# tahmidawal/Superresolution_for_PDEs

Measured on AMD Instinct MI355X. Metric: 20->40 SR training samples/sec at batch 1024 per GPU (fwd+MSE bwd+clip+AdamW), higher is better.
Workload: dtype f32 (h3: fp32 products from power-of-two-scaled 2-piece fp16 splits on fp16 MFMA, fp32 accumulate); 1 GPU; UNet 20->40 train step, fp32, batch 1024/GPU, 40x40; global_batch=1024, per_gpu_batch=1024, hw=40x40, parallelism=dp1

## Files before the change

include/srpde.h:

```cpp
#ifndef SRPDE_H_
#define SRPDE_H_

#include <stddef.h>

#ifdef __cplusplus
extern "C" {
#endif

typedef struct ihipStream_t* hipStream_t;

#define SRPDE_ABI_VERSION 17

#define SRPDE_FAM_NO_H5 2
#define SRPDE_FAM_NO_H4 4
#define SRPDE_FAM_NO_H3R 8

const char* srpde_last_error(void);
const char* srpde_last_kernel(void);
int srpde_version(void);

int srpde_pack_conv_weights(const float* w, float* wfwd, float* wdgrad, int cout, int cin, int cin_real,
                            int ksize, hipStream_t stream);
int srpde_conv_fwd(const float* x0, int c0, int ldx0, const float* x1, int c1, int ldx1, const float* wpack,
                   const float* bias, float* y, int ldy, int n, int h, int w, int cout, int ksize, int dil,
                   int sign, int accumulate, float* stats, const float* ep_mean, const float* ep_invstd,
                   const float* ep_gamma, const float* ep_beta, unsigned* ep_amax, void* workspace,
                   size_t ws_bytes, hipStream_t stream);
size_t srpde_conv_fwd_workspace_size(int cout);
size_t srpde_conv_stats_blocks(int n, int h, int w, int cout);
int srpde_conv_stats_rows_per_block(int cout);
size_t srpde_conv_wgrad_workspace_size(int n, int h, int w, int cout, int cin, int ksize);
int srpde_conv_wgrad(const float* dy, int lddy, const float* x0, int c0, int ldx0, const float* x1, int c1,
                     int ldx1, float* dw, int cin_real, int accumulate, int n, int h, int w, int cout, int ksize,
                     int dil, void* workspace, size_t ws_bytes, hipStream_t stream);
int srpde_conv_wgrad_bnb(const float* da, int ldda, const float* y, int ldy, const float* mean, const float* invstd,
                         const float* gamma, const float* beta, const float* m1, const float* m2, int flags,
                         const float* x0, int c0, int ldx0, float* dw, int cin_real, int accumulate, int n, int h,
                         int w, int cout, int ksize, int dil, void* workspace, size_t ws_bytes, hipStream_t stream);
int srpde_conv_h3_supported(int c0, int c1, int cout, int w, int dil, int ksize);
int srpde_conv_h3_stats_rows(void);
int srpde_conv_h3_stats_rows_for(int c0, int c1, int cout, int h, int w, int dil, int flags);
int srpde_split_weights_h3(const float* w, void* planes, int* wexp, int rows, int K, hipStream_t stream);
int srpde_absmax(const float* x, int ldx, int c, long long P, unsigned* amax, hipStream_t stream);
int srpde_prepare_weights_h3(const long long* desc, int nlayers, int total_rows, hipStream_t stream);
// ... 110 lines not shown
                                 const float* stats, int E, int S, int tile, float* x, hipStream_t stream);
int srpde_cascade_stitch_denorm(const float* y, const float* stats, int E, int S, int tile, double* u_next,
                                hipStream_t stream);
size_t srpde_field_metrics_workspace_size(int E, int n);
int srpde_field_metrics(const void* pred, int pred_is_f32, const double* gt, int E, int n, double* out,
                        void* workspace, size_t ws_bytes, hipStream_t stream);

int srpde_tiled_tiles_per_side(int S, int tile, int stride);
size_t srpde_tiled_level_stats_workspace_size(int E, int S);
int srpde_tiled_level_stats(const double* u_cur, const double* f_next, const double* theta_next, int E, int S,
                            float* stats, int* theta_const, void* workspace, size_t ws_bytes, hipStream_t stream);
int srpde_tiled_assemble(const double* u_cur, const double* f_next, const double* theta_next, const float* stats,
                         int E, int S, int tile, int stride, float* x, hipStream_t stream);
int srpde_tiled_blend_denorm(const float* y, const float* stats, int E, int S, int tile, int stride, int window,
                             double* u_next, hipStream_t stream);

int srpde_resize_bicubic_ac(const float* x, float* out, int planes, int h, int w, int ho, int wo,
                            hipStream_t stream);

int srpde_upsample_bilinear_fwd(const float* x, int ldx, float* out, int ldo, int n, int h, int w, int ho, int wo,
                                int c, hipStream_t stream);
int srpde_upsample_bilinear_bwd(const float* dout, int lddo, float* dx, int lddx, int n, int h, int w, int ho,
                                int wo, int c, int accumulate, hipStream_t stream);
int srpde_upsample_bilinear_gate_fwd(const float* x, int ldx, float* out, int ldo, int n, int h, int w, int ho,
                                      int wo, int c, const float* wg, const float* bg, float* sa, hipStream_t stream);
size_t srpde_upsample_gate_sa_workspace_size(int n, int h, int w);
int srpde_upsample_gate_sa(const float* x, int ldx, int n, int h, int w, int ho, int wo, int c, const float* wg,
                           const float* bg, float* sa, void* workspace, size_t ws_bytes, hipStream_t stream);
int srpde_conv_head_eval_supported(int w);
int srpde_conv_head_eval(const float* z, int ldz, const unsigned* amax_z, const void* wsplit, const int* wexp,
                         const float* bias, const float* bn_mean, const float* bn_invstd, const float* bn_gamma,
                         const float* bn_beta, const float* wf, const float* bf, const float* xin, int xin_c, int n,
                         int h, int w, float* out, hipStream_t stream);
int srpde_att_apply_fwd(const float* x, int ldx, int n, int hw, int c, const float* ca, const float* sa, float* out,
                        int ldo, hipStream_t stream);
int srpde_upsample_bilinear_bwd_gated(const float* dout, int lddo, const float* dsa, const float* wg, float* dx,
                                      int lddx, int n, int h, int w, int ho, int wo, int c, int accumulate,
                                      hipStream_t stream);
int srpde_gating_bn_reduce_blocks(long long P, int C);
int srpde_gating_bn_reduce(const float* dsa, const float* wg, float* dg, int lddg, const float* y, int ldy,
                           const float* mean, const float* invstd, const float* gamma, const float* beta, long long P,
                           int C, int flags, void* part, float* da_max, hipStream_t stream);
int srpde_upsample_bwd_bn_supported(int h, int w, int ho, int wo, int c, int lddo, int lddx);
int srpde_upsample_bilinear_bwd_gated_bn(const float* dout, int lddo, const float* dsa, const float* wg, float* dx,
                                         int lddx, int n, int h, int w, int ho, int wo, int c, const float* y, int ldy,
                                         const float* mean, const float* invstd, const float* gamma,
                                         const float* beta, int flags, void* part, float* da_max,
                                         hipStream_t stream);

int srpde_att_fwd(const float* x, int ldx, const float* g, int ldg, int n, int hw, int c, int gc, const float* w1,
                  const float* b1, const float* w2, const float* b2, const float* wg, const float* bg, float* m,
                  float* hbuf, float* ca, float* sa, float* out, int ldo, hipStream_t stream);
int srpde_att_channel_fwd(const float* x, int ldx, int n, int hw, int c, const float* w1, const float* b1,
                          const float* w2, const float* b2, float* m, float* hbuf, float* ca, hipStream_t stream);
int srpde_att_gate_fwd(const float* x, int ldx, const float* g, int ldg, int n, int hw, int c, int gc,
                       const float* ca, const float* wg, const float* bg, float* sa, float* out, int ldo,
                       hipStream_t stream);
size_t srpde_att_bwd_workspace_size(int n, int hw, int c, int gc);
int srpde_att_bwd(const float* dout, int lddo, const float* x, int ldx, const float* g, int ldg, int n, int hw,
                  int c, int gc, const float* w1, const float* w2, const float* wg, const float* m, const float* hbuf,
                  const float* ca, const float* sa, float* dx, int lddx, int dx_accumulate, float* dg, int lddg,
                  int dg_accumulate, float* dw1, float* db1, float* dw2, float* db2, float* dwg, float* dbg,
                  void* workspace, size_t ws_bytes, hipStream_t stream);
int srpde_att_pool_bn_bwd_blocks(int n, int h, int w, int c);
int srpde_att_pool_bn_bwd(const float* dout, int lddo, const float* ca, const float* sa, const float* dm, const float* a,
                          int lda, const float* dp, int lddp, const float* y, int ldy, const float* mean,
// ... 93 lines not shown
```

superresolution_for_pdes_amd/csrc/bn.hip:

```cpp
#include "bn_reduce.h"

namespace srpde {

struct Chan {
  double n, mean, m2;
};
__device__ __forceinline__ Chan chan_merge(Chan a, Chan b) {
  if (b.n == 0.0) return a;
  if (a.n == 0.0) return b;
  const double n = a.n + b.n, d = b.mean - a.mean;
  Chan r;
  r.n = n;
  r.mean = a.mean + d * (b.n / n);
  r.m2 = a.m2 + b.m2 + d * d * (a.n * b.n / n);
  return r;
}

__device__ __forceinline__ void fin_channel(int c, const float2* __restrict__ stats, int nblk, int nfull,
                                            int rows_per_blk, long long P, int C, double shift, double s1, double s2,
                                            double sm, float* running_mean, float* running_var, float momentum,
                                            float eps, float* __restrict__ mean_out, float* __restrict__ invstd_out,
                                            long long* num_batches_tracked, const float* __restrict__ gamma,
                                            const float* __restrict__ beta, float* __restrict__ scale_out,
                                            float* __restrict__ shift_out, unsigned* amax, float sqrt_pm1) {
// ... 306 lines not shown
      const float4 d = add4(scale4(dsa[p], w), old);
      st4(dg + p * lddg + c, d);
      acc.amax(d);
      acc.add(v, d, relu);
    };
    bn_rows(pb + r0, pe, rs, y, ldy, dg, lddg, c, row);
  }
  bn_bwd_block_combine(red4, threadIdx.x, (int)threadIdx.x < (C >> 2), threadIdx.x, C >> 2, rs, acc,
                       part + (size_t)blockIdx.x * C + c, true, da_max + blockIdx.x);
}

__global__ __launch_bounds__(256) void colsum2_kernel(const float2* __restrict__ part, int nblk, int C,
                                                      float* out0, float* out1, double* keep0, double* keep1) {
  const int c = blockIdx.x;
  __shared__ double a[256], b[256];
  double x = 0.0, yv = 0.0;
  for (int k = threadIdx.x; k < nblk; k += 256) {
    const float2 v = part[(size_t)k * C + c];
    x += v.x; yv += v.y;
  }
  a[threadIdx.x] = x; b[threadIdx.x] = yv;
  __syncthreads();
  for (int s = 128; s > 0; s >>= 1) {
    if ((int)threadIdx.x < s) { a[threadIdx.x] += a[threadIdx.x + s]; b[threadIdx.x] += b[threadIdx.x + s]; }
    __syncthreads();
  }
  if (threadIdx.x == 0) {
    if (out0) out0[c] = (float)a[0];
    if (out1) out1[c] = (float)b[0];
    if (keep0) keep0[c] = a[0];
    if (keep1) keep1[c] = b[0];
  }
}

struct BnBwdDy {
  float4 mu, is, g, b, m1, m2, k;
  __device__ __forceinline__ float dy1(float v, float mu1, float is1, float g1, float b1, float d, int relu, float a1,
                                       float a2, float k1) const {
    float xh;
    const float dz = bn_relu_mask(v, mu1, is1, g1, b1, d, relu, &xh);
    return (dz - a1 - xh * a2) * k1;
  }
  __device__ __forceinline__ float4 dy4(const float4& v, const float4& d, int relu) const {
    return make_float4(dy1(v.x, mu.x, is.x, g.x, b.x, d.x, relu, m1.x, m2.x, k.x),
                       dy1(v.y, mu.y, is.y, g.y, b.y, d.y, relu, m1.y, m2.y, k.y),
                       dy1(v.z, mu.z, is.z, g.z, b.z, d.z, relu, m1.z, m2.z, k.z),
                       dy1(v.w, mu.w, is.w, g.w, b.w, d.w, relu, m1.w, m2.w, k.w));
  }
};

__global__ __launch_bounds__(256) void bn_bwd_apply_kernel(const float* __restrict__ y, int ldy,
                                                           const float* __restrict__ da, int ldda,
                                                           const float* __restrict__ mean,
                                                           const float* __restrict__ invstd,
                                                           const float* __restrict__ gamma,
                                                           const float* __restrict__ beta,
                                                           const double* __restrict__ sdz,
                                                           const double* __restrict__ sdzx, long long P, int C,
                                                           int rows_per_blk, int relu, float* __restrict__ dy,
                                                           int lddy, float2* __restrict__ bias_part, unsigned* amax) {
  extern __shared__ float4 red4[];
  float mx = 0.f;
  int c4, r0, rs;
  thread_rc(C, &c4, &r0, &rs);
  const int active = (C >> 2) * rs;
  const int c = c4 * 4;
  float4 sb = zero4();
  if ((int)threadIdx.x < active) {
    const float4 mu = ld4(mean + c);
    const float4 is = ld4(invstd + c);
    const float4 g = ld4(gamma + c);
    const float4 b = ld4(beta + c);
    const double invP = (relu & 2) ? 0.0 : 1.0 / (double)P;
    float4 m1, m2, k;
    m1.x = (float)(sdz[c] * invP); m1.y = (float)(sdz[c + 1] * invP);
    m1.z = (float)(sdz[c + 2] * invP); m1.w = (float)(sdz[c + 3] * invP);
    m2.x = (float)(sdzx[c] * invP); m2.y = (float)(sdzx[c + 1] * invP);
    m2.z = (float)(sdzx[c + 2] * invP); m2.w = (float)(sdzx[c + 3] * invP);
    k.x = g.x * is.x; k.y = g.y * is.y; k.z = g.z * is.z; k.w = g.w * is.w;
    const long long pb = (long long)blockIdx.x * rows_per_blk;
    const long long pe = min(P, pb + rows_per_blk);
    const BnBwdDy f{mu, is, g, b, m1, m2, k};
// ... 639 lines not shown
```

superresolution_for_pdes_amd/csrc/bn_reduce.h:

```cpp
#pragma once
#include "vec4.h"

namespace srpde {

template <bool ALWAYS = false>
__device__ __forceinline__ float bn_relu_mask(float v, float mu, float is, float g, float b, float d, int relu,
                                              float* xhat) {
  const float xh = (v - mu) * is;
  *xhat = xh;
  return ((!ALWAYS && !(relu & 1)) || xh * g + b > 0.f) ? d : 0.f;
}

template <bool ALWAYS>
__device__ __forceinline__ void bn_bwd_add1(float v, float mu, float is, float g, float b, float d, int relu, float& t1,
                                            float& t2) {
  float xh;
  const float dz = bn_relu_mask<ALWAYS>(v, mu, is, g, b, d, relu, &xh);
  t1 += dz;
  t2 += dz * xh;
}

struct BnBwdAcc {
  float4 mu, is, g, b;
  float4 s1 = zero4(), s2 = zero4();
// ... 12 lines not shown
    bn_bwd_add1<ALWAYS>(y.y, mu.y, is.y, g.y, b.y, d.y, relu, s1.y, s2.y);
    bn_bwd_add1<ALWAYS>(y.z, mu.z, is.z, g.z, b.z, d.z, relu, s1.z, s2.z);
    bn_bwd_add1<ALWAYS>(y.w, mu.w, is.w, g.w, b.w, d.w, relu, s1.w, s2.w);
  }
  __device__ __forceinline__ void amax(const float4& d) { dmax = fmaxf(dmax, absmax4(d)); }
};

__device__ __forceinline__ void bn_bwd_store_part(const float4* sums, int C4, int nrows, int q, float2* o) {
  float4 t1 = zero4(), t2 = t1;
  for (int r = 0; r < nrows; ++r) {
    t1 = add4(t1, sums[r * C4 + q]);
    t2 = add4(t2, sums[256 + r * C4 + q]);
  }
  store_part4(o, t1, t2);
}
__device__ __forceinline__ float max4slots(const float* wmx) { return fmaxf(fmaxf(wmx[0], wmx[1]), fmaxf(wmx[2], wmx[3])); }

__device__ __forceinline__ void bn_bwd_block_combine(float4* red4, int tid, bool lead, int q, int C4, int nrows,
                                                     const BnBwdAcc& acc, float2* o, bool want_max, float* da_max) {
  red4[tid] = acc.s1;
  red4[256 + tid] = acc.s2;
  __syncthreads();
  if (lead) bn_bwd_store_part(red4, C4, nrows, q, o);
  if (want_max) {
    const float dmax = wave_max(acc.dmax);
    __syncthreads();
    float* wmx = reinterpret_cast<float*>(red4);
    if ((tid & 63) == 0) wmx[tid >> 6] = dmax;
    __syncthreads();
    if (tid == 0) *da_max = max4slots(wmx);
  }
}

}
```

superresolution_for_pdes_amd/csrc/conv_head.hip:

```cpp
#include "conv_h3.h"

namespace srpde {

struct HeadArgs {
  const float* z; int ldz;
  const unsigned* amax;
  const _Float16* wsp;
  const int* wexp;
  const float* bias;
  const float* mean; const float* invstd; const float* gamma; const float* beta;
  const float* wf; const float* bf;
  const float* xin; int xin_c;
  int N, H, W, P;
  float* out;
};

constexpr int HEAD_BM = 128, HEAD_SR = 160, HEAD_RB = HEAD_BM / 64;
constexpr int HEAD_IT = 4;

__global__ __launch_bounds__(256, 3) void conv_head_eval_kernel(HeadArgs a) {
  extern __shared__ __attribute__((aligned(16))) char lds[];
  const int tid = threadIdx.x, lane = tid & 63, wave = tid >> 6;
  const int l16 = lane & 15, lq = lane >> 4;
  const int W = a.W, HW = a.H * a.W, halo = W + 1, arows = HEAD_BM + 2 * halo;
  const int zrel = arows * HEAD_SR;
  const int m0 = blockIdx.x * HEAD_BM, pix0 = m0 - halo;
  const int ea = h3_exp(*a.amax);
  const float sa = exp2i(ea);

  half8 bh[9], bl[9];
#pragma unroll
  for (int t = 0; t < 9; ++t) {
    const size_t o = (size_t)l16 * 288 + t * 32 + lq * 8;
// ... 191 lines not shown
  float t = 0.f;
#pragma unroll
  for (int i = 0; i < HEAD_RB; ++i)
#pragma unroll
    for (int r = 0; r < 4; ++r) {
      const int px = m0 + wave * (16 * HEAD_RB) + i * 16 + lq * 4 + r;
      if (px < p.P) t += yv[i][r];
    }
  const float mean = chan_sum(t) / (float)cnt;
  t = 0.f;
#pragma unroll
  for (int i = 0; i < HEAD_RB; ++i)
#pragma unroll
    for (int r = 0; r < 4; ++r) {
      const int px = m0 + wave * (16 * HEAD_RB) + i * 16 + lq * 4 + r;
      const float d = yv[i][r] - mean;
      if (px < p.P) t = __builtin_fmaf(d, d, t);
    }
  const float m2 = chan_sum(t);
  if (tid < 16) p.stats[(size_t)blockIdx.x * 16 + tid] = make_float2(mean, m2);
}

bool n16_supported(int c0, int c1, int cout, int w, int dil) {
  return c0 == 32 && c1 == 0 && cout == 16 && dil == 1 && w > 0 && w <= 63 &&
         (size_t)(HEAD_BM + 2 * (w + 1)) * HEAD_SR + 128 + 256 <= 80 * 1024;
}

int launch_fwd_n16(const ConvParams& p, const H3Args& h, hipStream_t st) {
  const size_t lds = (size_t)(HEAD_BM + 2 * (p.W + 1)) * HEAD_SR + 128 + 256;
  note_kernel("conv_fwd_n16_kernel");
  hipLaunchKernelGGL(conv_fwd_n16_kernel, dim3(ceil_div(p.P, HEAD_BM)), dim3(256), lds, st, p, h);
  SRPDE_LAUNCH_CHECK("srpde_conv_fwd_h3(n16)");
  return 0;
}

}

using namespace srpde;

extern "C" {

int srpde_conv_head_eval_supported(int w) {
  return (w > 0 && w <= 63 && (size_t)(HEAD_BM + 2 * (w + 1)) * HEAD_SR + 128 <= 80 * 1024) ? 1 : 0;
}

int srpde_conv_head_eval(const float* z, int ldz, const unsigned* amax_z, const void* wsplit, const int* wexp,
                         const float* bias, const float* bn_mean, const float* bn_invstd, const float* bn_gamma,
                         const float* bn_beta, const float* wf, const float* bf, const float* xin, int xin_c, int n,
                         int h, int w, float* out, hipStream_t stream) {
  SRPDE_CHECK_ARG(z && amax_z && wsplit && wexp && bn_mean && bn_invstd && bn_gamma && bn_beta && wf && bf && xin &&
                      out && xin_c >= 1,
                  "srpde_conv_head_eval: null pointer");
  SRPDE_CHECK_ARG(n > 0 && h > 0 && w > 0 && (long long)n * h * w < (1LL << 31) && ldz % 4 == 0 && ldz >= 32 &&
                      aligned16(z) && aligned16(wsplit),
                  "srpde_conv_head_eval: bad shape / stride / alignment");
  HeadArgs a;
  a.z = z; a.ldz = ldz; a.amax = amax_z;
  a.wsp = static_cast<const _Float16*>(wsplit); a.wexp = wexp; a.bias = bias;
  a.mean = bn_mean; a.invstd = bn_invstd; a.gamma = bn_gamma; a.beta = bn_beta;
  a.wf = wf; a.bf = bf; a.xin = xin; a.xin_c = xin_c;
  a.N = n; a.H = h; a.W = w; a.P = n * h * w; a.out = out;
  const size_t lds = (size_t)(HEAD_BM + 2 * (w + 1)) * HEAD_SR + 128;
  SRPDE_CHECK_ARG(srpde_conv_head_eval_supported(w), "srpde_conv_head_eval: image rows too wide for the tile (w=%d > 63)",
                  w);
  note_kernel("conv_head_eval_kernel");
  hipLaunchKernelGGL(conv_head_eval_kernel, dim3(ceil_div(a.P, HEAD_BM)), dim3(256), lds, stream, a);
  SRPDE_LAUNCH_CHECK("srpde_conv_head_eval");
  return 0;
}

}
```

superresolution_for_pdes_amd/hipops.py:

```python
from __future__ import annotations

import os

import torch

from ._lib import call, last_error, query, stream_ptr

F32 = torch.float32


def _pl(t):
    assert t.dim() == 2 and (t.stride(1) == 1 or t.shape[1] == 1), "expected a [P, C] row-major view"
    assert t.dtype == F32 and t.is_cuda, "expected a CUDA fp32 tensor"
    return t.data_ptr(), t.stride(0)


def _p(t):
    return 0 if t is None else t.data_ptr()


def _pl_opt(t):
    return (0, 0, 0) if t is None else (*_pl(t), t.shape[1])


# ... 290 lines not shown
         beta.data_ptr(), P, C, flags, _p(part), part.shape[0] if part is not None else 0, _p(da_max),
         da_max.numel() if (part is not None) else 0, m1.data_ptr(), m2.data_ptr(), _p(dgamma), _p(dbeta), _p(dbias),
         word.data_ptr(), ws.data_ptr(), ws_bytes, stream_ptr())
    return m1, m2, word


def dx_max_slots(n, h, w, cin_dx, device):
    bn = 64 if cin_dx % 64 == 0 else 32
    return empty(-(-(n * h * w) // 256) * -(-cin_dx // bn), device=device)


def out_max_slots(n, h, w, cin, cout, dil, device):
    t = query("srpde_conv_h3_tiles", n * h * w, cin, cout, w, dil)
    assert t > 0, "out_max_slots: shape not on the h3 kernels"
    return empty(t, device=device)


def conv_dgrad_bnb(da, y, mean, invstd, gamma, beta, m1, m2, dy_amax, wpack, dx, n, h, w, cout_dy, cin_dx, dil,
                   dysplit, relu=True, bn_bwd=None, dx_max=None):
    planes, wexp = wpack.h3
    pda, ldda = _pl(da)
    py, ldy = _pl(y)
    pdx, lddx = _pl(dx)
    _check_rows(bn_bwd[5] if bn_bwd is not None else None, None, "the h3 kernel (bn_bwd_partials)")
    ws = _scratch(int(query("srpde_conv_fwd_workspace_size", cin_dx)), dx.device)
    _conv_call("srpde_conv_dgrad_h3_bnb", _conv_flop(cin_dx, cout_dy, 3, n, h, w), pda, ldda, dy_amax.data_ptr(), py,
               ldy, mean.data_ptr(), invstd.data_ptr(), gamma.data_ptr(), beta.data_ptr(), m1.data_ptr(),
               m2.data_ptr(), BN_RELU if relu else 0, planes.data_ptr(), wexp.data_ptr(), pdx, lddx, n, h, w, cout_dy,
               cin_dx, dil, dysplit.data_ptr(), *_bn_bwd_args(bn_bwd), _p(dx_max), ws.data_ptr(), ws.numel(),
               stream_ptr())
    dysplit._srpde_amax = dy_amax


def bn_bwd_partials(n, h, w, c, device):
    rows = int(query("srpde_conv_h3_stats_rows"))
    buf = empty(-(-(n * h * w) // rows), c, 2, device=device)
    buf._srpde_rows = rows
    return buf


class AmaxSlots:

    def __init__(self, n, device):
        self.buf = torch.zeros(n, dtype=torch.int32, device=device)
        self.next = 0
        self.eval_epilogue = False

    def take(self):
        if self.next >= self.buf.numel():
            raise RuntimeError("AmaxSlots exhausted")
        self.next += 1
        return self.buf[self.next - 1:self.next]


def tag_amax(t, slot):
    if slot is not None:
        t._srpde_amax = slot
    return t


def amax_of(x):
    a = getattr(x, "_srpde_amax", None)
    if a is None:
        a = torch.zeros(1, dtype=torch.int32, device=x.device)
        px, ld = _pl(x)
        call("srpde_absmax", px, ld, x.shape[1], x.shape[0], a.data_ptr(), stream_ptr())
# ... 735 lines not shown
```

superresolution_for_pdes_amd/unet_exec.py:

```python
from __future__ import annotations

import contextlib

import torch

from . import hipops as H

FORWARD_GROUPS = ["enc1", "enc2", "enc3", "bridge", "att3", "dec3", "att2", "dec2", "att1", "dec1",
                  "out_conv1", "out_bn1", "out_conv2", "out_bn2", "final"]
FLAT_GROUPS = list(reversed(FORWARD_GROUPS))


def flat_layout(model):
    named = dict(model.named_parameters())
    out, off = [], 0
    for grp in FLAT_GROUPS:
        for name, p in named.items():
            if name == grp or name.startswith(grp + "."):
                out.append((name, p, off, p.numel()))
                off += p.numel()
    assert off == sum(p.numel() for p in named.values()), "flat layout does not cover every parameter"
    return out


# ... 342 lines not shown
            fn()
        for t in keep:
            if t is not None:
                t.record_stream(self.side)

    def join(self):
        self.main.wait_stream(self.side)


_WGRAD_STREAM = True
_BWD_PRIORITY = "auto"
_PRIO_STREAMS = {}


def _priority_stream(dev):
    key = (dev.type, dev.index if dev.index is not None else torch.cuda.current_device())
    st = _PRIO_STREAMS.get(key)
    if st is None:
        lo, hi = torch.cuda.Stream.priority_range()
        st = _PRIO_STREAMS[key] = torch.cuda.Stream(device=dev, priority=hi)
    return st


def _xkeep(xp):
    return tuple(xp.tensors()) if isinstance(xp, H.XSource) else ()


def _bwd_path(saved, dx, dx_accumulate, cin, w, dil):
    x0, x1, y, _, _, xp, train = saved
    cout = y.shape[1]
    if (_FUSE_BN_APPLY and train and dx is not None and xp is not None and not dx_accumulate
            and cin <= _BNB_MAX_CIN and cout >= _BNB_MIN_COUT and H.bnb_capable(cout, cin, w, dil)):
        return "bnb"
    if (_PRESPLIT_BWD and train and dx is not None and xp is not None
            and H.h3_capable(H.cpad32(cout), 0, cin, w, dil)):
        return "presplit"
    if (_FUSE_WGRAD_BN and train and dx is None and xp is None and x0 is not None and x1 is None
            and x0.shape[1] % 32 != 0):
        return "wgrad_bnb"
    return "plain"


def _bn_prepare(conv, bn, saved, da, grads, part):
    _, _, y, mean, invstd, _, _ = saved
    part_t, da_max = part if part is not None else (None, None)
    return H.bn_bwd_prepare(y, da, mean, invstd, bn.weight, bn.bias, grads[bn.weight], grads[bn.bias],
                            grads[conv.bias], part=part_t, da_max=da_max)


def _below_reduction(below, n, h, w, cin, dev, max_slots):
    if below is None:
        return None, None, None
    bnb, sb = below
    out_part = H.bn_bwd_partials(n, h, w, cin, dev)
    bn_bwd = (sb[2], sb[3], sb[4], bnb.weight, bnb.bias, out_part)
    return bn_bwd, (max_slots() if max_slots is not None else None), out_part


def _submit(wq, fn, keep):
    if wq is None:
        fn()
    else:
        wq.submit(fn, keep)


def _cbr_bwd(conv, bn, saved, da, n, h, w, dil, grads, slots, dx=None, dx_accumulate=False, part=None,
             below=None, wq=None):
    x0, x1, y, mean, invstd, xp, train = saved
    P, cout = y.shape
    dev = y.device
    cin = conv.in_channels if x0 is None else x0.shape[1] + (x1.shape[1] if x1 is not None else 0)
    path = _bwd_path(saved, dx, dx_accumulate, cin, w, dil)
    if path in ("bnb", "presplit"):
        m1, m2, dyw = _bn_prepare(conv, bn, saved, da, grads, part)
        if path == "bnb":
            wd = _dgrad_weights(conv, cin, w, dil)
            dyp = H.split_planes_buffer(P, cout, dev)
            bn_bwd, dx_max, out_part = _below_reduction(below if _FUSE_BN_BWD else None, n, h, w, cin, dev,
                                                        lambda: H.dx_max_slots(n, h, w, cin, dev))
            H.conv_dgrad_bnb(da, y, mean, invstd, bn.weight, bn.bias, m1, m2, dyw, wd, dx, n, h, w, cout, cin, dil,
                             dyp, bn_bwd=bn_bwd, dx_max=dx_max)
        else:
            dyp = H.bn_bwd_apply_split(y, da, mean, invstd, bn.weight, bn.bias, m1, m2, dyw)
            _tap("dyp:" + getattr(conv, "_srpde_name", "?"), dyp)
            wd = _dgrad_weights(conv, cin, w, dil, cdy=H.cpad32(cout))
            bn_bwd, dx_max, out_part = _below_reduction(
                below if _FUSE_BN_BWD and not dx_accumulate else None, n, h, w, cin, dev,
                (lambda: H.out_max_slots(n, h, w, H.cpad32(cout), cin, dil, dev)) if _FUSE_BN_APPLY else None)
            H.conv_fwd_presplit(dyp, wd, None, dx, n, h, w, cin, 3, dil, -1, dx_accumulate, None, bn_bwd=bn_bwd,
                                out_max=dx_max)
        _tap_dgrad(conv, dyp, dx, dx_max, out_part)
        _submit(wq, lambda: H.conv_wgrad_h3p(dyp, xp, grads[conv.weight], n, h, w, 3, dil), (dyp, dyw) + _xkeep(xp))
        return None if out_part is None else (out_part, dx_max)
    dw = grads[conv.weight]
    if path == "wgrad_bnb":
        m1, m2, _ = _bn_prepare(conv, bn, saved, da, grads, part)
        _submit(wq, lambda: H.conv_wgrad_bnb(da, y, mean, invstd, bn.weight, bn.bias, m1, m2, x0, dw, n, h, w, 3, dil),
                (da, y, m1, m2))
        return None
    dy = H.empty(P, cout, device=dev)
    H.bn_relu_bwd(y, da, mean, invstd, bn.weight, bn.bias, dy, grads[bn.weight], grads[bn.bias], grads[conv.bias],
                  amax=slots.take(), part=part[0] if part is not None else None, eval_mode=not train)
    _tap("dy:" + getattr(conv, "_srpde_name", "?"), dy)
    dyp, out_part, dx_max = None, None, None
    if dx is not None:
# ... 364 lines not shown
```

Before: 36540 samples/s.

## Add fused narrow 16-channel conv backward path with BN-apply, dgrad and wgrad kernels

Adds a specialized backward path for 3x3 convs with 16 output and 32 input channels. One kernel fuses BN-backward apply, the fp16 two-piece split of dy, dgrad via MFMA and the reduction of the BN partials for the layer below. A second kernel computes wgrad from the stored dy split using transposed LDS reads. Both are meant to replace the generic padded-to-32 presplit path, cutting padding waste, separate apply/split passes and extra memory traffic for narrow layers. The cost is new specialized code and shape restrictions (w <= 63).

Result: no change. 36620 samples/s (median of 6 runs) (+0.2%).

```diff
diff --git a/include/srpde.h b/include/srpde.h
--- a/include/srpde.h
+++ b/include/srpde.h
@@ -9,7 +9,7 @@
 
 typedef struct ihipStream_t* hipStream_t;
 
-#define SRPDE_ABI_VERSION 17
+#define SRPDE_ABI_VERSION 18
 
 #define SRPDE_FAM_NO_H5 2
 #define SRPDE_FAM_NO_H4 4
@@ -186,6 +186,17 @@
                          const float* bias, const float* bn_mean, const float* bn_invstd, const float* bn_gamma,
                          const float* bn_beta, const float* wf, const float* bf, const float* xin, int xin_c, int n,
                          int h, int w, float* out, hipStream_t stream);
+int srpde_conv_bwd_n16_supported(int w, int cin, int cout, int dil);
+int srpde_conv_bwd_n16_dgrad(const float* da, int ldda, const float* y, int ldy, const float* mean,
+                             const float* invstd, const float* gamma, const float* beta, const float* m1,
+                             const float* m2, const unsigned* dy_amax, const void* wsplit, const int* wexp, float* dx,
+                             int lddx, int n, int h, int w, void* dysplit, const float* bn_y, int bn_ldy,
+                             const float* bn_mean, const float* bn_invstd, const float* bn_gamma, const float* bn_beta,
+                             void* bn_part, float* dx_max, hipStream_t stream);
+size_t srpde_conv_wgrad_n16_workspace_size(int n, int h, int w);
+int srpde_conv_wgrad_n16(const void* dysplit, const unsigned* amax_dy, const float* x, int ldx, const void* xsplit,
+                         const unsigned* amax_x, const float* in_scale, const float* in_shift, float* dw, int cin_real,
+                         int accumulate, int n, int h, int w, void* workspace, size_t ws_bytes, hipStream_t stream);
 int srpde_att_apply_fwd(const float* x, int ldx, int n, int hw, int c, const float* ca, const float* sa, float* out,
                         int ldo, hipStream_t stream);
 int srpde_upsample_bilinear_bwd_gated(const float* dout, int lddo, const float* dsa, const float* wg, float* dx,
diff --git a/superresolution_for_pdes_amd/csrc/bn.hip b/superresolution_for_pdes_amd/csrc/bn.hip
--- a/superresolution_for_pdes_amd/csrc/bn.hip
+++ b/superresolution_for_pdes_amd/csrc/bn.hip
@@ -362,22 +362,6 @@
     if (keep1) keep1[c] = b[0];
   }
 }
-
-struct BnBwdDy {
-  float4 mu, is, g, b, m1, m2, k;
-  __device__ __forceinline__ float dy1(float v, float mu1, float is1, float g1, float b1, float d, int relu, float a1,
-                                       float a2, float k1) const {
-    float xh;
-    const float dz = bn_relu_mask(v, mu1, is1, g1, b1, d, relu, &xh);
-    return (dz - a1 - xh * a2) * k1;
-  }
-  __device__ __forceinline__ float4 dy4(const float4& v, const float4& d, int relu) const {
-    return make_float4(dy1(v.x, mu.x, is.x, g.x, b.x, d.x, relu, m1.x, m2.x, k.x),
-                       dy1(v.y, mu.y, is.y, g.y, b.y, d.y, relu, m1.y, m2.y, k.y),
-                       dy1(v.z, mu.z, is.z, g.z, b.z, d.z, relu, m1.z, m2.z, k.z),
-                       dy1(v.w, mu.w, is.w, g.w, b.w, d.w, relu, m1.w, m2.w, k.w));
-  }
-};
 
 __global__ __launch_bounds__(256) void bn_bwd_apply_kernel(const float* __restrict__ y, int ldy,
                                                            const float* __restrict__ da, int ldda,
diff --git a/superresolution_for_pdes_amd/csrc/bn_reduce.h b/superresolution_for_pdes_amd/csrc/bn_reduce.h
--- a/superresolution_for_pdes_amd/csrc/bn_reduce.h
+++ b/superresolution_for_pdes_amd/csrc/bn_reduce.h
@@ -68,4 +68,20 @@
   }
 }
 
+struct BnBwdDy {
+  float4 mu, is, g, b, m1, m2, k;
+  __device__ __forceinline__ float dy1(float v, float mu1, float is1, float g1, float b1, float d, int relu, float a1,
+                                       float a2, float k1) const {
+    float xh;
+    const float dz = bn_relu_mask(v, mu1, is1, g1, b1, d, relu, &xh);
+    return (dz - a1 - xh * a2) * k1;
+  }
+  __device__ __forceinline__ float4 dy4(const float4& v, const float4& d, int relu) const {
+    return make_float4(dy1(v.x, mu.x, is.x, g.x, b.x, d.x, relu, m1.x, m2.x, k.x),
+                       dy1(v.y, mu.y, is.y, g.y, b.y, d.y, relu, m1.y, m2.y, k.y),
+                       dy1(v.z, mu.z, is.z, g.z, b.z, d.z, relu, m1.z, m2.z, k.z),
+                       dy1(v.w, mu.w, is.w, g.w, b.w, d.w, relu, m1.w, m2.w, k.w));
+  }
+};
+
 }
diff --git a/superresolution_for_pdes_amd/csrc/conv_head.hip b/superresolution_for_pdes_amd/csrc/conv_head.hip
--- a/superresolution_for_pdes_amd/csrc/conv_head.hip
+++ b/superresolution_for_pdes_amd/csrc/conv_head.hip
@@ -1,4 +1,5 @@
 #include "conv_h3.h"
+#include "bn_reduce.h"
 
 namespace srpde {
 
@@ -256,6 +257,417 @@
   hipLaunchKernelGGL(conv_fwd_n16_kernel, dim3(ceil_div(p.P, HEAD_BM)), dim3(256), lds, st, p, h);
   SRPDE_LAUNCH_CHECK("srpde_conv_fwd_h3(n16)");
   return 0;
+}
+
+
+struct N16BwdArgs {
+  const float* da; int ldda;
+  const float* y; int ldy;
+  const float* mean; const float* invstd; const float* gamma; const float* beta; const float* m1; const float* m2;
+  const unsigned* dy_amax;
+  const _Float16* wsp;
+  const int* wexp;
+  float* dx; int lddx;
+  _Float16* dyp;
+  const float* bn_y; int bn_ldy;
+  const float* bn_mean; const float* bn_invstd; const float* bn_gamma; const float* bn_beta;
+  float2* bn_part;
+  float* dx_max;
+  int H, W, P;
+};
+
+__device__ __forceinline__ float4 n16_ldc4(const float* p) { return make_float4(p[0], p[1], p[2], p[3]); }
+
+constexpr int N16_STG = 36;
+
+static size_t n16_bwd_lds(int w) {
+  return (size_t)2 * (HEAD_BM + 2 * (w + 1) + 1) * 32 + (size_t)4 * 32 * N16_STG * 4 + 4 * 64 * 4 + 64;
+}
+
+__global__ __launch_bounds__(256, 3) void conv_bwd_n16_dgrad_kernel(N16BwdArgs a) {
+  extern __shared__ __attribute__((aligned(16))) char lds[];
+  const int tid = threadIdx.x, lane = tid & 63, wave = tid >> 6;
+  const int l16 = lane & 15, lq = lane >> 4;
+  const int W = a.W, HW = a.H * a.W, halo = W + 1, arows = HEAD_BM + 2 * halo;
+  const int PL = (arows + 1) * 32;
+  char* img_lo = lds + PL;
+  float* stage = reinterpret_cast<float*>(lds + 2 * PL) + wave * (32 * N16_STG);
+  float* red = reinterpret_cast<float*>(lds + 2 * PL + 4 * 32 * N16_STG * 4);
+  const int m0 = blockIdx.x * HEAD_BM, pix0 = m0 - halo;
+  const int ea = h3_exp(*a.dy_amax);
+  const float sa = exp2i(ea);
+
+  const int c8 = tid & 1;
+  if (tid < 16) {
+    reinterpret_cast<unsigned*>(lds + arows * 32)[tid & 7] = 0u;
+    reinterpret_cast<unsigned*>(img_lo + arows * 32)[tid & 7] = 0u;
+  }
+  float4 vd[2][2], vy[2][2];
+#pragma unroll
+  for (int k = 0; k < 2; ++k) {
+    const int r = (tid + 256 * k) >> 1, pix = pix0 + r;
+    vd[k][0] = vd[k][1] = vy[k][0] = vy[k][1] = make_float4(0.f, 0.f, 0.f, 0.f);
+    if (r < arows && pix >= 0 && pix < a.P) {
+      vd[k][0] = *reinterpret_cast<const float4*>(a.da + (size_t)pix * a.ldda + c8 * 8);
+      vd[k][1] = *reinterpret_cast<const float4*>(a.da + (size_t)pix * a.ldda + c8 * 8 + 4);
+      vy[k][0] = *reinterpret_cast<const float4*>(a.y + (size_t)pix * a.ldy + c8 * 8);
+      vy[k][1] = *reinterpret_cast<const float4*>(a.y + (size_t)pix * a.ldy + c8 * 8 + 4);
+    }
+  }
+  {
+    BnBwdDy f[2];
+#pragma unroll
+    for (int q = 0; q < 2; ++q) {
+      const int c = c8 * 8 + q * 4;
+      f[q].mu = n16_ldc4(a.mean + c); f[q].is = n16_ldc4(a.invstd + c); f[q].g = n16_ldc4(a.gamma + c);
+      f[q].b = n16_ldc4(a.beta + c);
+      f[q].m1 = n16_ldc4(a.m1 + c); f[q].m2 = n16_ldc4(a.m2 + c);
+      f[q].k = make_float4(f[q].g.x * f[q].is.x, f[q].g.y * f[q].is.y, f[q].g.z * f[q].is.z, f[q].g.w * f[q].is.w);
+    }
+    const size_t dplane = (size_t)a.P * 16;
+#pragma unroll
+    for (int k = 0; k < 2; ++k) {
+      const int r = (tid + 256 * k) >> 1, pix = pix0 + r;
+      if (r < arows) {
+        half8 hv = {0, 0, 0, 0, 0, 0, 0, 0}, lv = {0, 0, 0, 0, 0, 0, 0, 0};
+        const bool inside = pix >= 0 && pix < a.P;
+        if (inside) split2h(f[0].dy4(vy[k][0], vd[k][0], 1), f[1].dy4(vy[k][1], vd[k][1], 1), sa, hv, lv);
+        *reinterpret_cast<half8*>(lds + r * 32 + c8 * 16) = hv;
+        *reinterpret_cast<half8*>(img_lo + r * 32 + c8 * 16) = lv;
+        if (inside && r >= halo && r < halo + HEAD_BM) {
+          _Float16* o = a.dyp + (size_t)pix * 16 + c8 * 8;
+          *reinterpret_cast<half8*>(o) = hv;
+          *reinterpret_cast<half8*>(o + dplane) = lv;
+        }
+      }
+    }
+  }
+  half8 bh[5][2], bl[5][2];
+#pragma unroll
+  for (int s = 0; s < 5; ++s)
+#pragma unroll
+    for (int j = 0; j < 2; ++j) {
+      const int tap = 2 * s + (lq >> 1);
+      bh[s][j] = bl[s][j] = half8{0, 0, 0, 0, 0, 0, 0, 0};
+      if (tap < 9) {
+        const size_t o = (size_t)(16 * j + l16) * 288 + tap * 32 + (lq & 1) * 8;
+        bh[s][j] = *reinterpret_cast<const half8*>(a.wsp + o);
+        bl[s][j] = *reinterpret_cast<const half8*>(a.wsp + 32 * 288 + o);
+      }
+    }
+  int we[2];
+  we[0] = a.wexp[l16]; we[1] = a.wexp[16 + l16];
+  __syncthreads();
+
+  floatx4 acc[HEAD_RB][2];
+#pragma unroll
+  for (int i = 0; i < HEAD_RB; ++i) {
+    const int rr = wave * (16 * HEAD_RB) + i * 16 + l16;
+    const int m = m0 + rr;
+    int yy = -(1 << 20), xx = 0;
+    if (m < a.P) {
+      const int rem = m % HW;
+      yy = rem / W;
+      xx = rem - yy * W;
+    }
+    acc[i][0] = acc[i][1] = floatx4{0.f, 0.f, 0.f, 0.f};
+#pragma unroll
+    for (int s = 0; s < 5; ++s) {
+      const int t0 = 2 * s, t1 = 2 * s + 1;
+      const int ky = (lq >> 1) ? t1 / 3 : t0 / 3, kx = (lq >> 1) ? t1 % 3 : t0 % 3;
+      const int iy = yy + 1 - ky, ix = xx + 1 - kx;
+      const bool ok = (t1 < 9 || !(lq >> 1)) && iy >= 0 && iy < a.H && ix >= 0 && ix < W;
+      const int o = ok ? (rr + (2 - ky) * W + (2 - kx)) * 32 + (lq & 1) * 16 : arows * 32;
+      const half8 ah = *reinterpret_cast<const half8*>(lds + o);
+      const half8 al = *reinterpret_cast<const half8*>(img_lo + o);
+#pragma unroll
+      for (int j = 0; j < 2; ++j) {
+        floatx4 c0 = __builtin_amdgcn_mfma_f32_16x16x32_f16(al, bh[s][j], acc[i][j], 0, 0, 0);
+        c0 = __builtin_amdgcn_mfma_f32_16x16x32_f16(ah, bl[s][j], c0, 0, 0, 0);
+        acc[i][j] = __builtin_amdgcn_mfma_f32_16x16x32_f16(ah, bh[s][j], c0, 0, 0, 0);
+      }
+    }
+  }
+#pragma unroll
+  for (int j = 0; j < 2; ++j) {
+    const int e = ea + we[j];
+    const bool wide = e > 126 || e < -126;
+    const float ia = exp2i(-ea), cs = wide ? exp2i(-we[j]) : exp2i(-e);
+#pragma unroll
+    for (int i = 0; i < HEAD_RB; ++i)
+#pragma unroll
+      for (int r = 0; r < 4; ++r)
+        stage[(i * 16 + lq * 4 + r) * N16_STG + 16 * j + l16] = (wide ? acc[i][j][r] * ia : acc[i][j][r]) * cs;
+  }
+  __syncthreads();
+  const int c4 = (lane & 7) * 4;
+  const bool bnr = a.bn_part != nullptr;
+  float4 mu = zero4(), is = zero4(), ga = zero4(), be = zero4();
+  if (bnr) {
+    mu = n16_ldc4(a.bn_mean + c4); is = n16_ldc4(a.bn_invstd + c4);
+    ga = n16_ldc4(a.bn_gamma + c4); be = n16_ldc4(a.bn_beta + c4);
+  }
+  float4 v[4], yv[4];
+#pragma unroll
+  for (int it = 0; it < 4; ++it) {
+    const int row = it * 8 + (lane >> 3), px = m0 + wave * 32 + row;
+    v[it] = *reinterpret_cast<const float4*>(stage + row * N16_STG + c4);
+    yv[it] = zero4();
+    if (px < a.P) {
+      *reinterpret_cast<float4*>(a.dx + (size_t)px * a.lddx + c4) = v[it];
+      if (bnr) yv[it] = *reinterpret_cast<const float4*>(a.bn_y + (size_t)px * a.bn_ldy + c4);
+    }
+  }
+  float mx = 0.f;
+  float4 s1 = zero4(), s2 = zero4();
+#pragma unroll
+  for (int it = 0; it < 4; ++it) {
+    const int px = m0 + wave * 32 + it * 8 + (lane >> 3);
+    if (px < a.P) {
+      mx = fmaxf(mx, absmax4(v[it]));
+      float xh, dz;
+#define N16_BNP(X)                                              \
+  xh = (yv[it].X - mu.X) * is.X;                                \
+  dz = __builtin_fmaf(xh, ga.X, be.X) > 0.f ? v[it].X : 0.f;    \
+  s1.X += dz;                                                   \
+  s2.X = __builtin_fmaf(dz, xh, s2.X);
+      N16_BNP(x) N16_BNP(y) N16_BNP(z) N16_BNP(w)
+#undef N16_BNP
+    }
+  }
+#pragma unroll
+  for (int o = 8; o < 64; o <<= 1) {
+    s1.x += __shfl_xor(s1.x, o, 64); s1.y += __shfl_xor(s1.y, o, 64);
+    s1.z += __shfl_xor(s1.z, o, 64); s1.w += __shfl_xor(s1.w, o, 64);
+    s2.x += __shfl_xor(s2.x, o, 64); s2.y += __shfl_xor(s2.y, o, 64);
+    s2.z += __shfl_xor(s2.z, o, 64); s2.w += __shfl_xor(s2.w, o, 64);
+  }
+#pragma unroll
+  for (int o = 32; o > 0; o >>= 1) mx = fmaxf(mx, __shfl_xor(mx, o, 64));
+  if (lane < 8) {
+    float* rw = red + wave * 64;
+    rw[c4] = s1.x; rw[c4 + 1] = s1.y; rw[c4 + 2] = s1.z; rw[c4 + 3] = s1.w;
+    rw[32 + c4] = s2.x; rw[32 + c4 + 1] = s2.y; rw[32 + c4 + 2] = s2.z; rw[32 + c4 + 3] = s2.w;
+  }
+  if (lane == 0) red[256 + wave] = mx;
+  __syncthreads();
+  if (bnr && tid < 32) {
+    const float t1 = (red[tid] + red[64 + tid]) + (red[128 + tid] + red[192 + tid]);
+    const float t2 = (red[32 + tid] + red[96 + tid]) + (red[160 + tid] + red[224 + tid]);
+    a.bn_part[(size_t)blockIdx.x * 32 + tid] = make_float2(t1, t2);
+  }
+  if (a.dx_max != nullptr && tid == 0)
+    a.dx_max[blockIdx.x] = fmaxf(fmaxf(red[256], red[257]), fmaxf(red[258], red[259]));
+}
+
+struct N16WgArgs {
+  const _Float16* dyp; const unsigned* ady;
+  const float* x; int ldx; const unsigned* ax;
+  const _Float16* xp;
+  const float* in_scale; const float* in_shift;
+  float* part;
+  int H, W, P, ntiles, tiles_per;
+};
+constexpr int N16W_FOLD = 8;
+
+static size_t n16_wg_xbytes(int w) { return std::max((size_t)2 * (HEAD_BM + 2 * (w + 1)) * 64, (size_t)64 * 72 * 4); }
+static size_t n16_wg_lds(int w) { return n16_wg_xbytes(w) + 2 * HEAD_BM * 32 + HEAD_BM; }
+
+typedef short n16_v4i16 __attribute__((ext_vector_type(4)));
+typedef unsigned n16_u4 __attribute__((ext_vector_type(4)));
+
+template <int RB>
+__device__ __forceinline__ half8 n16_tr(const char* img, int row0, int colbyte, int l16) {
+  const int o = (row0 + (l16 >> 2)) * RB + colbyte + (l16 & 3) * 8;
+  const n16_v4i16 p = __builtin_amdgcn_ds_read_tr16_b64_v4i16(
+      (__attribute__((address_space(3))) n16_v4i16*)(uintptr_t)lds_addr_of(img + o));
+  const n16_v4i16 q = __builtin_amdgcn_ds_read_tr16_b64_v4i16(
+      (__attribute__((address_space(3))) n16_v4i16*)(uintptr_t)lds_addr_of(img + o + 4 * RB));
+  typedef short v8i16 __attribute__((ext_vector_type(8)));
+  const v8i16 c = {p.x, p.y, p.z, p.w, q.x, q.y, q.z, q.w};
+  return __builtin_bit_cast(half8, c);
+}
+
+__global__ __launch_bounds__(256, 2) void conv_wgrad_n16_kernel(N16WgArgs a) {
+  extern __shared__ __attribute__((aligned(16))) char lds[];
+  const int tid = threadIdx.x, lane = tid & 63, wave = tid >> 6;
+  const int l16 = lane & 15, lq = lane >> 4;
+  const int W = a.W, HW = a.H * a.W, halo = W + 1, arows = HEAD_BM + 2 * halo;
+  char* xh = lds;
+  char* xl = lds + arows * 64;
+  char* dyh = lds + (int)max(2 * (HEAD_BM + 2 * (W + 1)) * 64, 64 * 72 * 4);
+  char* dyl = dyh + HEAD_BM * 32;
+  unsigned char* flags = reinterpret_cast<unsigned char*>(dyl + HEAD_BM * 32);
+  const int ea = h3_exp(*a.ady), eb = h3_exp(*a.ax);
+  const float sb = exp2i(eb);
+  const size_t dplane = (size_t)a.P * 16;
+
+  floatx4 acc[9][2], part[9][2];
+#pragma unroll
+  for (int t = 0; t < 9; ++t)
+#pragma unroll
+    for (int j = 0; j < 2; ++j) acc[t][j] = part[t][j] = floatx4{0.f, 0.f, 0.f, 0.f};
+
+  const int t_begin = blockIdx.x * a.tiles_per, t_end = min(a.ntiles, t_begin + a.tiles_per);
+  int nfold = 0;
+  for (int tile = t_begin; tile < t_end; ++tile) {
+    const int m0 = tile * HEAD_BM, pix0 = m0 - halo;
+    __syncthreads();
+    {
+      float4 v[HEAD_IT][2];
+      const bool planes = a.x == nullptr;
+      const size_t xplane = (size_t)a.P * 32;
+#pragma unroll
+      for (int k = 0; k < HEAD_IT; ++k) {
+        const int sg = tid + 256 * k, r = sg >> 2, c8 = sg & 3;
+        const int pix = pix0 + r;
+        v[k][0] = v[k][1] = make_float4(0.f, 0.f, 0.f, 0.f);
+        if (planes) {
+          if (r < arows && pix >= 0 && pix < a.P) {
+            v[k][0] = *reinterpret_cast<const float4*>(a.xp + (size_t)pix * 32 + c8 * 8);
+            v[k][1] = *reinterpret_cast<const float4*>(a.xp + xplane + (size_t)pix * 32 + c8 * 8);
+          }
+        } else if (r < arows && pix >= 0 && pix < a.P) {
+          v[k][0] = *reinterpret_cast<const float4*>(a.x + (size_t)pix * a.ldx + c8 * 8);
+          v[k][1] = *reinterpret_cast<const float4*>(a.x + (size_t)pix * a.ldx + c8 * 8 + 4);
+        }
+      }
+      half8 dh = {0, 0, 0, 0, 0, 0, 0, 0}, dl = {0, 0, 0, 0, 0, 0, 0, 0};
+      {
+        const int pix = m0 + (tid >> 1);
+        if (pix < a.P) {
+          const _Float16* o = a.dyp + (size_t)pix * 16 + (tid & 1) * 8;
+          dh = *reinterpret_cast<const half8*>(o);
+          dl = *reinterpret_cast<const half8*>(o + dplane);
+        }
+      }
+#pragma unroll
+      for (int k = 0; k < HEAD_IT; ++k) {
+        const int sg = tid + 256 * k, r = sg >> 2, c8 = sg & 3;
+        if (r < arows && planes) {
+          *reinterpret_cast<float4*>(xh + r * 64 + c8 * 16) = v[k][0];
+          *reinterpret_cast<float4*>(xl + r * 64 + c8 * 16) = v[k][1];
+        } else if (r < arows) {
+          const int pix = pix0 + r;
+          const bool inside = pix >= 0 && pix < a.P;
+          float4 a0 = v[k][0], a1 = v[k][1];
+          if (a.in_scale != nullptr) {
+            const float4 s0 = n16_ldc4(a.in_scale + c8 * 8), s1 = n16_ldc4(a.in_scale + c8 * 8 + 4);
+            const float4 t0 = n16_ldc4(a.in_shift + c8 * 8), t1 = n16_ldc4(a.in_shift + c8 * 8 + 4);
+#define N16_AFF(V, S, T, X) V.X = inside ? fmaxf(V.X * S.X + T.X, 0.f) : 0.f;
+            N16_AFF(a0, s0, t0, x) N16_AFF(a0, s0, t0, y) N16_AFF(a0, s0, t0, z) N16_AFF(a0, s0, t0, w)
+            N16_AFF(a1, s1, t1, x) N16_AFF(a1, s1, t1, y) N16_AFF(a1, s1, t1, z) N16_AFF(a1, s1, t1, w)
+#undef N16_AFF
+          }
+          half8 hv, lv;
+          split2h(a0, a1, sb, hv, lv);
+          *reinterpret_cast<half8*>(xh + r * 64 + c8 * 16) = hv;
+          *reinterpret_cast<half8*>(xl + r * 64 + c8 * 16) = lv;
+        }
+      }
+      *reinterpret_cast<half8*>(dyh + (tid >> 1) * 32 + (tid & 1) * 16) = dh;
+      *reinterpret_cast<half8*>(dyl + (tid >> 1) * 32 + (tid & 1) * 16) = dl;
+      if (tid < HEAD_BM) {
+        const int p = m0 + tid;
+        unsigned f = 0xfu;
+        if (p < a.P) {
+          const int rem = p % HW, yy = rem / W, xx = rem - yy * W;
+          f = (yy == 0 ? 1u : 0u) | (yy == a.H - 1 ? 2u : 0u) | (xx == 0 ? 4u : 0u) | (xx == W - 1 ? 8u : 0u);
+        }
+        flags[tid] = (unsigned char)f;
+      }
+    }
+    __syncthreads();
+    const int kb = wave * 32 + 8 * lq;
+    const half8 ah = n16_tr<32>(dyh, kb, 0, l16), al = n16_tr<32>(dyl, kb, 0, l16);
+    const unsigned f0 = *reinterpret_cast<const unsigned*>(flags + kb);
+    const unsigned f1 = *reinterpret_cast<const unsigned*>(flags + kb + 4);
+#pragma unroll
+    for (int t = 0; t < 9; ++t) {
+      const int ky = t / 3, kx = t % 3;
+      const unsigned bm = (ky == 0 ? 1u : 0u) | (ky == 2 ? 2u : 0u) | (kx == 0 ? 4u : 0u) | (kx == 2 ? 8u : 0u);
+      half8 ahm = ah, alm = al;
+      if (bm != 0u) {
+        n16_u4 mk;
+#define N16_MK(F, SH) ((((F) >> (SH)) & bm) ? 0u : 0xffffu)
+        mk.x = N16_MK(f0, 0) | (N16_MK(f0, 8) << 16);
+        mk.y = N16_MK(f0, 16) | (N16_MK(f0, 24) << 16);
+        mk.z = N16_MK(f1, 0) | (N16_MK(f1, 8) << 16);
+        mk.w = N16_MK(f1, 16) | (N16_MK(f1, 24) << 16);
+#undef N16_MK
+        ahm = __builtin_bit_cast(half8, __builtin_bit_cast(n16_u4, ah) & mk);
+        alm = __builtin_bit_cast(half8, __builtin_bit_cast(n16_u4, al) & mk);
+      }
+#pragma unroll
+      for (int j = 0; j < 2; ++j) {
+        const half8 bh = n16_tr<64>(xh, kb + ky * W + kx, j * 32, l16);
+        const half8 bl = n16_tr<64>(xl, kb + ky * W + kx, j * 32, l16);
+        floatx4 c0 = __builtin_amdgcn_mfma_f32_16x16x32_f16(alm, bh, part[t][j], 0, 0, 0);
+        c0 = __builtin_amdgcn_mfma_f32_16x16x32_f16(ahm, bl, c0, 0, 0, 0);
+        part[t][j] = __builtin_amdgcn_mfma_f32_16x16x32_f16(ahm, bh, c0, 0, 0, 0);
+      }
+    }
+    if (++nfold == N16W_FOLD) {
+      nfold = 0;
+#pragma unroll
+      for (int t = 0; t < 9; ++t)
+#pragma unroll
+        for (int j = 0; j < 2; ++j) {
+          acc[t][j] += part[t][j];
+          part[t][j] = floatx4{0.f, 0.f, 0.f, 0.f};
+        }
+    }
+  }
+  const float ia = exp2i(-ea), ib = exp2i(-eb);
+#pragma unroll
+  for (int t = 0; t < 9; ++t)
+#pragma unroll
+    for (int j = 0; j < 2; ++j) {
+      acc[t][j] += part[t][j];
+#pragma unroll
+      for (int r = 0; r < 4; ++r) acc[t][j][r] = (acc[t][j][r] * ia) * ib;
+    }
+  float* rbuf = reinterpret_cast<float*>(lds);
+  for (int wv = 1; wv < 4; ++wv) {
+    __syncthreads();
+    if (wave == wv) {
+#pragma unroll
+      for (int t = 0; t < 9; ++t)
+#pragma unroll
+        for (int j = 0; j < 2; ++j)
+#pragma unroll
+          for (int r = 0; r < 4; ++r) rbuf[((t * 2 + j) * 4 + r) * 64 + lane] = acc[t][j][r];
+    }
+    __syncthreads();
+    if (wave == 0) {
+#pragma unroll
+      for (int t = 0; t < 9; ++t)
+#pragma unroll
+        for (int j = 0; j < 2; ++j)
+#pragma unroll
+          for (int r = 0; r < 4; ++r) acc[t][j][r] += rbuf[((t * 2 + j) * 4 + r) * 64 + lane];
+    }
+  }
+  if (wave == 0) {
+    float* slab = a.part + (size_t)blockIdx.x * (16 * 288);
+#pragma unroll
+    for (int t = 0; t < 9; ++t)
+#pragma unroll
+      for (int j = 0; j < 2; ++j)
+#pragma unroll
+        for (int r = 0; r < 4; ++r) slab[(4 * lq + r) * 288 + t * 32 + 16 * j + l16] = acc[t][j][r];
+  }
+}
+
+bool n16_bwd_supported(int w, int cin, int cout, int dil) {
+  return cin == 32 && cout == 16 && dil == 1 && w > 0 && w <= 63 && n16_bwd_lds(w) <= 64 * 1024 &&
+         n16_wg_lds(w) <= 64 * 1024;
+}
+
+static void n16_wg_plan(int P, int* ntiles, int* tiles_per, int* grid) {
+  *ntiles = ceil_div(P, HEAD_BM);
+  *tiles_per = ceil_div(*ntiles, std::min(*ntiles, 2 * cu_count()));
+  *grid = ceil_div(*ntiles, *tiles_per);
 }
 
 }
@@ -293,4 +705,79 @@
   return 0;
 }
 
-}
+int srpde_conv_bwd_n16_supported(int w, int cin, int cout, int dil) { return n16_bwd_supported(w, cin, cout, dil) ? 1 : 0; }
+
+int srpde_conv_bwd_n16_dgrad(const float* da, int ldda, const float* y, int ldy, const float* mean,
+                             const float* invstd, const float* gamma, const float* beta, const float* m1,
+                             const float* m2, const unsigned* dy_amax, const void* wsplit, const int* wexp, float* dx,
+                             int lddx, int n, int h, int w, void* dysplit, const float* bn_y, int bn_ldy,
+                             const float* bn_mean, const float* bn_invstd, const float* bn_gamma, const float* bn_beta,
+                             void* bn_part, float* dx_max, hipStream_t stream) {
+  SRPDE_CHECK_ARG(da && y && mean && invstd && gamma && beta && m1 && m2 && dy_amax && wsplit && wexp && dx && dysplit,
+                  "srpde_conv_bwd_n16_dgrad: null pointer");
+  SRPDE_CHECK_ARG(bn_part == nullptr || (bn_y && bn_mean && bn_invstd && bn_gamma && bn_beta),
+                  "srpde_conv_bwd_n16_dgrad: null pointer (the fused BN reduction needs bn_y / mean / invstd / gamma / beta)");
+  SRPDE_CHECK_ARG(n > 0 && h > 0 && n16_bwd_supported(w, 32, 16, 1) && (long long)n * h * w < (1LL << 26),
+                  "srpde_conv_bwd_n16_dgrad: shape not supported (n=%d h=%d w=%d; needs w <= 63)", n, h, w);
+  SRPDE_CHECK_ARG(ldda % 4 == 0 && ldda >= 16 && ldy % 4 == 0 && ldy >= 16 && lddx % 4 == 0 && lddx >= 32 &&
+                      (bn_part == nullptr || (bn_ldy % 4 == 0 && bn_ldy >= 32)),
+                  "srpde_conv_bwd_n16_dgrad: row strides must be multiples of 4 and hold the channels");
+  SRPDE_CHECK_ARG(aligned16(da) && aligned16(y) && aligned16(dx) && aligned16(dysplit) && aligned16(wsplit) &&
+                      (bn_part == nullptr || (aligned16(bn_y) && aligned16(bn_part))),
+                  "srpde_conv_bwd_n16_dgrad: da, y, dx, dysplit, wsplit, bn_y and bn_part must be 16-byte aligned");
+  N16BwdArgs a;
+  a.da = da; a.ldda = ldda; a.y = y; a.ldy = ldy;
+  a.mean = mean; a.invstd = invstd; a.gamma = gamma; a.beta = beta; a.m1 = m1; a.m2 = m2; a.dy_amax = dy_amax;
+  a.wsp = static_cast<const _Float16*>(wsplit); a.wexp = wexp;
+  a.dx = dx; a.lddx = lddx; a.dyp = static_cast<_Float16*>(dysplit);
+  a.bn_y = bn_y; a.bn_ldy = bn_ldy; a.bn_mean = bn_mean; a.bn_invstd = bn_invstd; a.bn_gamma = bn_gamma;
+  a.bn_beta = bn_beta; a.bn_part = static_cast<float2*>(bn_part); a.dx_max = dx_max;
+  a.H = h; a.W = w; a.P = n * h * w;
+  note_kernel("conv_bwd_n16_dgrad_kernel");
+  hipLaunchKernelGGL(conv_bwd_n16_dgrad_kernel, dim3(ceil_div(a.P, HEAD_BM)), dim3(256), n16_bwd_lds(w), stream, a);
+  SRPDE_LAUNCH_CHECK("srpde_conv_bwd_n16_dgrad");
+  return 0;
+}
+
+size_t srpde_conv_wgrad_n16_workspace_size(int n, int h, int w) {
+  if (n <= 0 || h <= 0 || w <= 0) return 0;
+  int ntiles, tiles_per, grid;
+  n16_wg_plan(n * h * w, &ntiles, &tiles_per, &grid);
+  return (size_t)grid * 16 * 288 * sizeof(float);
+}
+
+int srpde_conv_wgrad_n16(const void* dysplit, const unsigned* amax_dy, const float* x, int ldx, const void* xsplit,
+                         const unsigned* amax_x, const float* in_scale, const float* in_shift, float* dw, int cin_real,
+                         int accumulate, int n, int h, int w, void* workspace, size_t ws_bytes, hipStream_t stream) {
+  SRPDE_CHECK_ARG(dysplit && amax_dy && (x || xsplit) && amax_x && dw && workspace, "srpde_conv_wgrad_n16: null pointer");
+  SRPDE_CHECK_ARG((x == nullptr) != (xsplit == nullptr), "srpde_conv_wgrad_n16: the input is x or xsplit, not both");
+  SRPDE_CHECK_ARG((in_scale == nullptr) == (in_shift == nullptr) && (in_scale == nullptr || x != nullptr),
+                  "srpde_conv_wgrad_n16: in_scale / in_shift go together (and with x: a stored split has them applied)");
+  SRPDE_CHECK_ARG(n > 0 && h > 0 && n16_bwd_supported(w, 32, 16, 1) && (long long)n * h * w < (1LL << 26) &&
+                      cin_real > 0 && cin_real <= 32,
+                  "srpde_conv_wgrad_n16: shape not supported (n=%d h=%d w=%d cin_real=%d; needs w <= 63)", n, h, w,
+                  cin_real);
+  SRPDE_CHECK_ARG(x == nullptr || (ldx % 4 == 0 && ldx >= 32),
+                  "srpde_conv_wgrad_n16: ldx must be a multiple of 4 and >= 32");
+  SRPDE_CHECK_ARG(aligned16(dysplit) && aligned16(x) && aligned16(xsplit) && aligned16(workspace),
+                  "srpde_conv_wgrad_n16: dysplit, x / xsplit and workspace must be 16-byte aligned");
+  N16WgArgs a;
+  int grid;
+  a.P = n * h * w;
+  n16_wg_plan(a.P, &a.ntiles, &a.tiles_per, &grid);
+  if (ws_bytes < (size_t)grid * 16 * 288 * sizeof(float)) {
+    set_error("srpde_conv_wgrad_n16: workspace %zu < %zu bytes", ws_bytes, (size_t)grid * 16 * 288 * sizeof(float));
+    return kErrWorkspace;
+  }
+  a.dyp = static_cast<const _Float16*>(dysplit); a.ady = amax_dy;
+  a.x = x; a.ldx = ldx; a.xp = static_cast<const _Float16*>(xsplit); a.ax = amax_x; a.in_scale = in_scale; a.in_shift = in_shift;
+  a.part = static_cast<float*>(workspace);
+  a.H = h; a.W = w;
+  note_kernel("conv_wgrad_n16_kernel");
+  hipLaunchKernelGGL(conv_wgrad_n16_kernel, dim3(grid), dim3(256), n16_wg_lds(w), stream, a);
+  SRPDE_LAUNCH_CHECK("srpde_conv_wgrad_n16");
+  return wgrad_reduce(a.part, dw, grid, 16, 32, cin_real, 9, accumulate, stream);
+}
+
+
+}
diff --git a/superresolution_for_pdes_amd/hipops.py b/superresolution_for_pdes_amd/hipops.py
--- a/superresolution_for_pdes_amd/hipops.py
+++ b/superresolution_for_pdes_amd/hipops.py
@@ -346,6 +346,50 @@
     dysplit._srpde_amax = dy_amax
 
 
+def conv_bwd_n16_supported(w, cin, cout, dil, pixels=None):
+    return (_CONV_MATH == "h3" and (pixels is None or pixels >= 4096)
+            and bool(query("srpde_conv_bwd_n16_supported", w, cin, cout, dil)))
+
+
+def n16_blocks(n, h, w):
+    return -(-(n * h * w) // 128)
+
+
+def conv_bwd_n16_dgrad(da, y, mean, invstd, gamma, beta, m1, m2, dy_amax, wpack, dx, n, h, w, bn_bwd=None,
+                       dx_max=None, dysplit=None):
+    planes, wexp = wpack.h3
+    P = y.shape[0]
+    pda, ldda = _pl(da)
+    py, ldy = _pl(y)
+    pdx, lddx = _pl(dx)
+    if dysplit is None:
+        dysplit = split_planes_buffer(P, 16, y.device)
+    if bn_bwd is not None:
+        _check_rows(bn_bwd[5], 128, "srpde_conv_bwd_n16_dgrad")
+    _conv_call("srpde_conv_bwd_n16_dgrad", _conv_flop(32, 16, 3, n, h, w), pda, ldda, py, ldy, mean.data_ptr(),
+               invstd.data_ptr(), gamma.data_ptr(), beta.data_ptr(), m1.data_ptr(), m2.data_ptr(), dy_amax.data_ptr(),
+               planes.data_ptr(), wexp.data_ptr(), pdx, lddx, n, h, w, dysplit.data_ptr(), *_bn_bwd_args(bn_bwd),
+               _p(dx_max), stream_ptr())
+    dysplit._srpde_amax = dy_amax
+    return dysplit
+
+
+def conv_wgrad_n16(dyp, xs, dw, n, h, w, accumulate=False):
+    assert dyp.shape[2] == 16
+    if isinstance(xs, XSource):
+        assert xs.x1 is None and xs.x1_gate is None
+        (p0, ld0), pxp, ax, aff = _pl(xs.x0), 0, xs.a0, xs.in_affine
+    else:
+        assert xs.shape[2] == 32 and not isinstance(xs._srpde_amax, tuple)
+        p0, ld0, pxp, ax, aff = 0, 0, xs.data_ptr(), xs._srpde_amax, None
+    ws_bytes = int(query("srpde_conv_wgrad_n16_workspace_size", n, h, w))
+    ws = torch.empty(max(ws_bytes, 16), dtype=torch.uint8, device=dyp.device)
+    _conv_call("srpde_conv_wgrad_n16", _conv_flop(16, dw.shape[1], 3, n, h, w), dyp.data_ptr(),
+               dyp._srpde_amax.data_ptr(), p0, ld0, pxp, ax.data_ptr(), _p(aff[0] if aff else None),
+               _p(aff[1] if aff else None), dw.data_ptr(), dw.shape[1], int(accumulate), n, h, w, ws.data_ptr(),
+               ws_bytes, stream_ptr())
+
+
 def bn_bwd_partials(n, h, w, c, device):
     rows = int(query("srpde_conv_h3_stats_rows"))
     buf = empty(-(-(n * h * w) // rows), c, 2, device=device)
diff --git a/superresolution_for_pdes_amd/unet_exec.py b/superresolution_for_pdes_amd/unet_exec.py
--- a/superresolution_for_pdes_amd/unet_exec.py
+++ b/superresolution_for_pdes_amd/unet_exec.py
@@ -398,6 +398,12 @@
     if (_FUSE_BN_APPLY and train and dx is not None and xp is not None and not dx_accumulate
             and cin <= _BNB_MAX_CIN and cout >= _BNB_MIN_COUT and H.bnb_capable(cout, cin, w, dil)):
         return "bnb"
+    if (_PRESPLIT_BWD and train and dx is not None and not dx_accumulate and xp is not None
+            and (xp.x1 is None and xp.x1_gate is None if isinstance(xp, H.XSource)
+                 else not isinstance(xp._srpde_amax, tuple))
+            and H.conv_bwd_n16_supported(w, cin, cout, dil, y.shape[0])
+            and H.h3_capable(H.cpad32(cout), 0, cin, w, dil)):
+        return "n16"
     if (_PRESPLIT_BWD and train and dx is not None and xp is not None
             and H.h3_capable(H.cpad32(cout), 0, cin, w, dil)):
         return "presplit"
@@ -437,6 +443,20 @@
     dev = y.device
     cin = conv.in_channels if x0 is None else x0.shape[1] + (x1.shape[1] if x1 is not None else 0)
     path = _bwd_path(saved, dx, dx_accumulate, cin, w, dil)
+    if path == "n16":
+        m1, m2, dyw = _bn_prepare(conv, bn, saved, da, grads, part)
+        wd = _dgrad_weights(conv, cin, w, dil, cdy=H.cpad32(cout))
+        bn_bwd, dx_max, out_part = None, None, None
+        if below is not None and _FUSE_BN_BWD:
+            out_part = H.empty(H.n16_blocks(n, h, w), cin, 2, device=dev)
+            out_part._srpde_rows = 128
+            bn_bwd = (below[1][2], below[1][3], below[1][4], below[0].weight, below[0].bias, out_part)
+            dx_max = H.empty(H.n16_blocks(n, h, w), device=dev) if _FUSE_BN_APPLY else None
+        dyp = H.conv_bwd_n16_dgrad(da, y, mean, invstd, bn.weight, bn.bias, m1, m2, dyw, wd, dx, n, h, w,
+                                   bn_bwd=bn_bwd, dx_max=dx_max)
+        _tap_dgrad(conv, dyp, dx, dx_max, out_part)
+        _submit(wq, lambda: H.conv_wgrad_n16(dyp, xp, grads[conv.weight], n, h, w), (dyp, dyw) + _xkeep(xp))
+        return None if out_part is None else (out_part, dx_max)
     if path in ("bnb", "presplit"):
         m1, m2, dyw = _bn_prepare(conv, bn, saved, da, grads, part)
         if path == "bnb":
```
